# ArielElb/zkSnark-FinalProject

Measured on AMD Instinct MI355X. Metric: groth16_proofs_per_sec, higher is better.
Workload: dtype u32; 1 GPU; matrix-mul 128x128 + Poseidon MatrixCircuit: 10706932 constraints, 8675313 witness vars, domain 2^24; pk/R1CS/assignment resident in HBM; real key (zkg16_setup_resident) with window tables (zkg16_pk_precompute), last timed proof verified (zkg16_verify); parallelism=1 GPU

## Files before the change

__graft_entry__.py:

```python
import os
import subprocess
import sys

ROOT = os.path.dirname(os.path.abspath(__file__))
for p in (ROOT, os.path.join(ROOT, "tests"), os.path.join(ROOT, "tests", "golden"), os.path.join(ROOT, "oracle")):
    if p not in sys.path:
        sys.path.insert(0, p)


def build():
    import importlib.util
    spec = importlib.util.spec_from_file_location("zkg16_build", os.path.join(ROOT, "zksnark-finalproject_amd", "build.py"))
    mod = importlib.util.module_from_spec(spec)
    spec.loader.exec_module(mod)
    mod.build()
    subprocess.check_call(["make", "-C", os.path.join(ROOT, "oracle"), "-s"])
    import prim_cases
    prim_cases.build_shim("host")
    prim_cases.build_shim("device")
    import madd_lazy_cases
    madd_lazy_cases.build_shim("host")
    madd_lazy_cases.build_shim("device")
    import zksnark_finalproject_amd as z
    z.load()
    return None


def smoke():
    import random

    import numpy as np

    import oracle as orc
    import synth
    from helpers import fr_mont, fr_mont_vec
    import pyref as P
    from zksnark_finalproject_amd import Device

    dev = Device(0)
    rng = random.Random(2026)
    nc, ni, nv = 3000, 4, 2500
    A, B, C, z = synth.random_r1cs(rng, nc, ni, nv)
    r1cs = synth.r1cs_arrays(A, B, C, ni)
    pk, _ = synth.make_pk(orc, r1cs, nv, rng, point_gen=dev.fixed_base)
    zm = fr_mont_vec(z)
    r, s = fr_mont(P.rand_fr(rng)), fr_mont(P.rand_fr(rng))
    ph = dev.pk_load(pk, ni)
    proof, inf = dev.prove(ph, r, s, r1cs, zm)
    eproof, einf = orc.prove(pk, r, s, r1cs, zm)
    assert np.array_equal(proof, eproof) and np.array_equal(inf, einf), "HIP proof != oracle proof"
    print("smoke ok: proof bit-identical to the oracle;", dev.last_timings())
    dev.close()
    return None


if __name__ == "__main__":
    build()
    if len(sys.argv) > 1 and sys.argv[1] == "smoke":
        smoke()
```

zksnark-finalproject_amd/build.py:

```python
import os
import subprocess
import sys
from concurrent.futures import ThreadPoolExecutor

HERE = os.path.dirname(os.path.abspath(__file__))
CSRC = os.path.join(HERE, "csrc")
OBJ = os.path.join(HERE, "build")
LIB = os.path.join(HERE, "libzkg16.so")
SOURCES = ["api.hip", "api_keys.hip", "api_prove.hip", "api_stages.hip", "api_group.hip", "api_verify.hip", "api_rerandomize.hip", "api_trapdoor.hip", "ntt.hip", "poly.hip", "msm.hip", "sort.hip", "bucket_sort.hip", "setup.hip", "circuits.hip", "verify.hip", "witness.hip", "matrix_r1cs.hip", "prime_device.hip", "group.hip", "verify_batch.hip"]
HEADERS = ["ff.cuh", "ffu.cuh", "fru.cuh", "ec.cuh", "common.hpp", "api_internal.hpp", "hostff.hpp", "matrix_plan.hpp", "prime_program.hpp", "group.hpp", "verify_batch.hpp", "pairing_dev.cuh", "pairing_each_dev.cuh", "decompress_dev.cuh", "sponge_chain_dev.cuh", "linear_dev.cuh", "linear_elim_dev.cuh", "prime_inputs_dev.cuh", "u64_inputs_dev.cuh", "rerandomize_dev.cuh", "r1cs_check_dev.cuh", "trapdoor_dev.cuh", "pairing_fast.inc", "poseidon_h64.inc", "poseidon_params.inc", "prime_circuit.inc", "final_exp.inc", os.path.join("..", "..", "include", "zkg16.h")]
FLAGS = ["--offload-arch=gfx950", "-O3", "-std=c++17", "-fPIC", "-fvisibility=hidden", "-Wall", "-Wno-unused-function"]


def _stale(target, deps):
    if not os.path.exists(target):
        return True
    t = os.path.getmtime(target)
    return any(os.path.getmtime(d) > t for d in deps)


def build(force=False, verbose=True):
    os.makedirs(OBJ, exist_ok=True)
    hdrs = [os.path.join(CSRC, h) for h in HEADERS] + [os.path.abspath(__file__)]
    jobs = []
    for src in SOURCES:
        s = os.path.join(CSRC, src)
        o = os.path.join(OBJ, src.replace(".hip", ".o"))
        if force or _stale(o, [s] + hdrs):
            jobs.append((s, o))

    def cc(job):
        s, o = job
        cmd = ["hipcc"] + FLAGS + ["-c", s, "-o", o]
        if verbose:
            print(" ".join(cmd), flush=True)
        subprocess.check_call(cmd)

    with ThreadPoolExecutor(max_workers=4) as ex:
        list(ex.map(cc, jobs))
    objs = [os.path.join(OBJ, s.replace(".hip", ".o")) for s in SOURCES]
    if force or jobs or _stale(LIB, objs):
        cmd = ["hipcc", "--offload-arch=gfx950", "-shared", "-fPIC", "-o", LIB] + objs
        if verbose:
            print(" ".join(cmd), flush=True)
        subprocess.check_call(cmd)
    return LIB


if __name__ == "__main__":
    build(force="--force" in sys.argv)
```

zksnark-finalproject_amd/csrc/api.hip:

```cpp
#include "api_internal.hpp"

using namespace zk;

namespace zk {
ScopedKernelTimer::ScopedKernelTimer(zkg16_ctx *c, const char *n, double u, hipStream_t st)
    : ctx(c), name(n), units(u), stream(st ? st : c->stream) {
    if (!ctx->opt.kernel_timing) return;
    if (ctx->opt.kernel_timing_accumulate_only && strncmp(n, "msm_accumulate", 14) != 0) return;
    ZK_HIP(hipEventCreate(&e0));
    ZK_HIP(hipEventCreate(&e1));
    ZK_HIP(hipEventRecord(e0, stream));
}
ScopedKernelTimer::~ScopedKernelTimer() {
    if (!e0) return;
    (void)hipEventRecord(e1, stream);
    ctx->pending_events.push_back(PendingEvent{name, units, e0, e1});
}
void kernel_timer_resolve(zkg16_ctx *ctx) {
    if (ctx->pending_events.empty()) return;
    (void)hipStreamSynchronize(ctx->stream);
    (void)hipStreamSynchronize(ctx->wm_stream);
    for (auto &sl : ctx->slots)
        if (sl.stream) (void)hipStreamSynchronize(sl.stream);
    for (auto &p : ctx->pending_events) {
// ... 278 lines not shown
    if (!ctx) return;
    (void)hipSetDevice(ctx->device);
    for (auto &l : ctx->lanes)
        if (l) {
            {
                std::lock_guard<std::mutex> lk(l->mu);
                teardown(l.get());
            }
            l.reset();
        }
    teardown(ctx);
    ctx->pks.clear();
    ctx->r1cs.clear();
    ctx->wits.clear();
    ctx->prime_dev.reset();
    ctx->ntt_tables.clear();
    delete ctx;
    dev_cache_flush();
}

}
namespace {
int set_option_one(zkg16_ctx *ctx, const char *name, int64_t v) {
    zkg16_ctx::Options &o = ctx->opt;
    const auto is = [name](const char *n) { return !strcmp(name, n); };
    const auto set = [v](int &dst, int64_t lo, int64_t hi, int64_t stored, bool also = true) {
        if (v < lo || v > hi || !also) return (int)ZKG16_ERR_BAD_ARG;
        dst = (int)stored;
        return (int)ZKG16_OK;
    };
    if (is("window_bits")) return set(o.window_bits, 0, 20, v, v != 1);
    if (is("min_seg")) return set(o.min_seg, 0, 4096, v);
    if (is("ntt_mode")) return set(o.ntt_mode, 0, 3, v, v != 2);
    if (is("reduce_mode")) return set(o.reduce_mode, 0, 6, v == 0 ? 3 : v == 4 ? 0 : v);
    if (is("g1_waves")) return set(o.g1_waves, 0, 4, v);
    if (is("fixup_aux")) return set(o.fixup_aux, INT64_MIN, INT64_MAX, v ? 1 : 0);
    if (is("window_bits_h")) return set(o.window_bits_h, 0, 20, v, v != 1);
    if (is("wm_concurrent")) { o.wm_concurrent = (int)v; return ZKG16_OK; }
    if (is("ntt_radix")) return set(o.ntt_radix, 0, 4, v == 0 ? 1 : v);
    if (is("ntt_xcd")) return set(o.ntt_xcd, 0, 2, v == 2 ? 0 : 1);
    if (is("table_stride")) return set(o.table_stride, 0, 2, v);
    if (is("acc_debug")) return set(o.acc_debug, 0, 15, v);
    if (is("sort_mode")) return set(o.sort_mode, 0, 1, v);
    if (is("acc_pipeline")) return set(o.acc_pipeline, 0, 4, v == 4 ? 0 : v);
    if (is("fuse_pointwise")) return set(o.fuse_pointwise, INT64_MIN, INT64_MAX, v ? 1 : 0);
    if (is("wm_transforms")) return set(o.wm_transforms, 0, 7, v == 7 ? 7 : 6, v == 0 || v >= 6);
    if (is("wm_first")) return set(o.wm_first, -1, 2, v);
    if (is("spmv_dict")) return set(o.spmv_dict, 0, 2, v);
    if (is("b_filter")) return set(o.b_filter, 0, 2, v);
    if (is("collect_threads")) return set(o.collect_threads, 0, 2, v == 0 ? -1 : v == 2 ? 0 : 1);
    if (is("fixed_base_bits")) return set(o.fixed_base_bits, 0, 20, v, v == 0 || (v >= 4 && !(v > 14 && (v & 1))));
    if (is("g2_lazy")) return set(o.g2_lazy, 0, 2, v == 2 ? 0 : 1);
    if (is("g1_inline")) return set(o.g1_inline, 0, 2, v == 2 ? 0 : 1);
    if (is("acc_lazy")) return set(o.acc_lazy, 0, 1, v);
    if (is("matrix_parts")) return set(o.matrix_parts, 0, 8, v);
    if (is("matrix_slice_min")) return set(o.matrix_slice_min, 0, 1 << 20, v == 0 ? MATRIX_SLICE_MIN_DEFAULT : v);
    if (is("batch_max")) return set(o.batch_max, 0, 65535, v);
    if (is("matrix_batch_threads")) return set(o.matrix_batch_threads, 0, 16, v);
    if (is("matrix_batch_grid")) return set(o.matrix_batch_grid, 0, 65535, v);
    if (is("linear_solver")) return set(o.linear_solver, 0, 1, v);
    if (is("linear_elim_lds_max")) return set(o.linear_elim_lds_max, 0, 64, v);
    if (is("sponge_chains_min")) {
        if (v < 0) return ZKG16_ERR_BAD_ARG;
        o.sponge_chains_min = v == 0 ? ZKG16_SPONGE_CHAINS_MIN_DEFAULT : v;
        return ZKG16_OK;
    }
    if (is("sponge_chain_segment")) return set(o.sponge_chain_segment, 0, 65535, v);
    if (is("verify_batch_min")) return set(o.verify_batch_min, 0, 1 << 30, v == 0 ? ZKG16_VERIFY_BATCH_MIN_DEFAULT : v);
    if (is("verify_wire_min")) return set(o.verify_wire_min, 0, 1 << 30, v == 0 ? ZKG16_VERIFY_WIRE_MIN_DEFAULT : v);
    if (is("verify_each_after")) {
        const int rc = set(o.verify_each_after, 0, 1 << 30, v == 0 ? ZKG16_VERIFY_EACH_AFTER_DEFAULT : v);
        if (rc == ZKG16_OK) o.verify_each_after_set = v != 0;
        return rc;
    }
    if (is("rerandomize_min")) return set(o.rerandomize_min, 0, 1 << 30, v == 0 ? ZKG16_RERANDOMIZE_MIN_DEFAULT : v);
    if (is("rerandomize_pass")) return set(o.rerandomize_pass, 0, 65536, v);
    if (is("check_satisfied")) return set(o.check_satisfied, 0, 1, v);
    if (is("trapdoor_pass")) return set(o.trapdoor_pass, 0, 65535, v);
    if (is("reduce_chunk")) return set(o.reduce_chunk, 0, 64, v, (v & (v - 1)) == 0);
    return ZKG16_ERR_UNSUPPORTED;
}
}
extern "C" {

int zkg16_set_option(zkg16_ctx *ctx, const char *name, int64_t value) {
    if (!ctx || !name) return ZKG16_ERR_BAD_ARG;
    if (!strcmp(name, "lanes")) {
        if (value < 1 || value > 8) return ZKG16_ERR_BAD_ARG;
        std::lock_guard<std::mutex> lk(ctx->lane_mu);
        ctx->opt_lanes = (int)value;
        return ZKG16_OK;
    }
    int rc;
    {
        std::lock_guard<std::mutex> lk(ctx->mu);
        rc = set_option_one(ctx, name, value);
    }
    if (rc != ZKG16_OK) return rc;
    std::vector<zkg16_ctx *> ls;
    {
        std::lock_guard<std::mutex> lk(ctx->lane_mu);
        for (auto &l : ctx->lanes)
            if (l) ls.push_back(l.get());
    }
    for (zkg16_ctx *l : ls) {
        std::lock_guard<std::mutex> lk(l->mu);
// ... 174 lines not shown
```

zksnark-finalproject_amd/csrc/common.hpp:

```cpp
#pragma once
#include <hip/hip_runtime.h>
#include <stdint.h>
#include <stdio.h>
#include <string.h>

#include <algorithm>
#include <array>
#include <atomic>
#include <condition_variable>
#include <functional>
#include <map>
#include <memory>
#include <mutex>
#include <shared_mutex>
#include <string>
#include <system_error>
#include <thread>
#include <vector>

#include "../../include/zkg16.h"
#include "ec.cuh"
#include "ff.cuh"

namespace zk {
// ... 218 lines not shown
    zkg16_ctx *root = nullptr;
    std::unique_ptr<zkg16_ctx> lanes[7];
    std::mutex lane_mu;
    std::condition_variable lane_cv;
    bool lane_busy[8] = {false, false, false, false, false, false, false, false};
    int opt_lanes = 2;
    int last_lane = 0;
    std::shared_mutex key_rw;
    struct LaneLogEntry { int lane; double t0_ms, t1_ms; };
    std::vector<LaneLogEntry> lane_log;
    zk::MsmWorkspace ws_z, ws_h, ws_zb;
    hipStream_t wm_stream = nullptr;
    zk::MsmSlot slots[5];
    int last_msm_group = 0;
    void *extra_host = nullptr;
    void *stage_host[2] = {nullptr, nullptr};
    hipEvent_t stage_done[2] = {nullptr, nullptr};
    zk::DevBuf poly[4];
    void *batch_host = nullptr;
    size_t batch_host_bytes = 0;
    bool batch_terms_set = false;
    uint64_t batch_terms[3] = {0, 0, 0};
    void *mbatch_host = nullptr;
    size_t mbatch_host_bytes = 0;
    zk::DevBuf mbatch_dev;
    zk::DevBuf check_dev;
    std::vector<uint64_t> check_n_bad, check_first_bad;
    float timings[zk::PROOF_TIMING_SLOTS] = {0};
    struct Options {
        bool kernel_timing = false;
        bool kernel_timing_accumulate_only = false;
        int window_bits = 0;
        int min_seg = 0;
        int ntt_mode = 1;
        int reduce_mode = 3;
        int b_filter = 0;
        int spmv_dict = 0;
        int wm_first = -1;
        int g1_waves = 0;
        int fixup_aux = 0;
        int window_bits_h = 0;
        int reduce_chunk = 0;
        int wm_concurrent = -1;
        int ntt_radix = 1;
        int ntt_xcd = 1;
        int table_stride = 0;
        int acc_debug = 0;
        int sort_mode = 0;
        int acc_pipeline = 0;
        int collect_threads = -1;
        int fixed_base_bits = 0;
        int g2_lazy = 1;
        int acc_lazy = 1;
        int g1_inline = 1;
        int matrix_parts = 0;
        int matrix_slice_min = MATRIX_SLICE_MIN_DEFAULT;
        int fuse_pointwise = 1;
        int wm_transforms = 6;
        int batch_max = 0;
        int matrix_batch_threads = 0;
        int matrix_batch_grid = 0;
        int linear_solver = 0;
        int linear_elim_lds_max = 0;
        int64_t sponge_chains_min = ZKG16_SPONGE_CHAINS_MIN_DEFAULT;
        int sponge_chain_segment = 0;
        int verify_batch_min = ZKG16_VERIFY_BATCH_MIN_DEFAULT;
        int verify_wire_min = ZKG16_VERIFY_WIRE_MIN_DEFAULT;
        int check_satisfied = 0;
        int verify_each_after = ZKG16_VERIFY_EACH_AFTER_DEFAULT;
        int rerandomize_min = ZKG16_RERANDOMIZE_MIN_DEFAULT;
        int rerandomize_pass = 0;
        int trapdoor_pass = 0;
        int verify_each_after_set = 0;
    } opt;
    std::map<std::string, zk::KernelStat> kstats;
    std::vector<zk::PendingEvent> pending_events;
    void *circuit_stage = nullptr;
    size_t circuit_stage_bytes = 0;
    float vb_timings[zk::VERIFY_TIMING_SLOTS] = {0};
    float rr_timings[zk::RERANDOMIZE_TIMING_SLOTS] = {0};
    int num_cus = 256;
    bool lds_attr_fixup[2] = {false, false}, lds_attr_ntt = false, lds_attr_linear_elim = false;
    zk::FixedBaseCache fb_g1, fb_g2;
    zk::DevBuf poseidon_dev;
    std::shared_ptr<zk::PrimeDev> prime_dev;
};

namespace zk {

struct PendingEvent { std::string name; double units; hipEvent_t e0, e1; };

struct ScopedKernelTimer {
    zkg16_ctx *ctx;
    const char *name;
    double units;
    hipEvent_t e0 = nullptr, e1 = nullptr;
    hipStream_t stream;
    ScopedKernelTimer(zkg16_ctx *c, const char *n, double u, hipStream_t st = nullptr);
    ~ScopedKernelTimer();
};
void kernel_timer_resolve(zkg16_ctx *ctx);

struct NttPointwise { const Fr *b, *c; Fr zinv; };
struct NttLast { const Fr *scale; bool pw_operand, sub; };
Fr *ntt_run(zkg16_ctx *ctx, Fr *src, Fr *dst, int log_n, bool inverse, bool coset, const NttPointwise *pw = nullptr,
            const NttLast *last = nullptr);
// ... 151 lines not shown
```

zksnark-finalproject_amd/csrc/msm.hip:

```cpp
#include <chrono>

#include "common.hpp"

namespace zk {

template <class F> struct FieldTraits;
template <> struct FieldTraits<FqU> { using Sat = Fq; static constexpr bool g2 = false; };
template <> struct FieldTraits<Fq2U> { using Sat = Fq2; static constexpr bool g2 = true; };
template <> struct FieldTraits<Fq> { using Sat = Fq; static constexpr bool g2 = false; };
template <> struct FieldTraits<Fq2> { using Sat = Fq2; static constexpr bool g2 = true; };

template <class T>
__device__ __forceinline__ T ldv(const T *p) {
    static_assert(sizeof(T) % 16 == 0, "16-byte multiple");
    T v;
    const uint4 *q = reinterpret_cast<const uint4 *>(p);
    uint4 *d = reinterpret_cast<uint4 *>(&v);
#pragma unroll
    for (unsigned i = 0; i < sizeof(T) / 16; i++) d[i] = q[i];
    return v;
}
template <class T>
__device__ __forceinline__ void stv(T *p, const T &v) {
    uint4 *q = reinterpret_cast<uint4 *>(p);
    const uint4 *s = reinterpret_cast<const uint4 *>(&v);
#pragma unroll
    for (unsigned i = 0; i < sizeof(T) / 16; i++) q[i] = s[i];
}

struct DigitSrc {
    const uint32_t *scalars, *extra;
    size_t n_main, n;
    const uint8_t *mask;
    int mont;
    const uint8_t *part;
    int want;
    const uint32_t *const *vecs;
    size_t vec_stride;
};
__global__ void __launch_bounds__(256) msm_digits_kernel(DigitSrc src, int c, int nwin, size_t nb, uint64_t *keys, uint32_t *codes, uint32_t invalid_bucket) {
    const size_t i = (size_t)blockIdx.x * blockDim.x + threadIdx.x;
    const size_t n = src.n;
    if (i >= n) return;
    const unsigned v = blockIdx.y;
    const uint32_t *mainv = src.vecs ? src.vecs[v] : src.scalars + (size_t)v * src.vec_stride * 8;
    const uint32_t *extrav = src.extra + (size_t)v * (n - src.n_main) * 8;
    const size_t w0 = (size_t)v * nwin;
    uint32_t s[9];
    {
        const uint4 *q = reinterpret_cast<const uint4 *>(i < src.n_main ? mainv + 8 * i : extrav + 8 * (i - src.n_main));
        uint4 lo = q[0], hi = q[1];
        if (src.mask && src.mask[i]) lo = hi = make_uint4(0, 0, 0, 0);
        if (src.part && (int)src.part[i] != src.want) lo = hi = make_uint4(0, 0, 0, 0);
        Fr v;
        v.l[0] = lo.x; v.l[1] = lo.y; v.l[2] = lo.z; v.l[3] = lo.w; v.l[4] = hi.x; v.l[5] = hi.y; v.l[6] = hi.z; v.l[7] = hi.w;
// ... 189 lines not shown
                    head_b = (int32_t)cur;
                    dst = a.seg_head + t;
                } else if (!acc.is_inf()) {
                    dst = a.buckets + cur;
                }
                if (dst != nullptr && !(a.debug & 1u)) stv(dst, acc);
                acc = XYZZ<F>::inf();
                cur = gb;
            }
            const Affine<F> b = bq;
            en = en1;
            en1 = a.entries[p + 2 < end ? p + 2 : end - 1];
            bq = ld_base<F>(bases, (a.debug & 2u) ? 0u : (a.debug & 4u) ? ((en.x >> 1) & 0xffffu) : (en.x >> 1));
            __builtin_amdgcn_sched_barrier(0);
            if constexpr (LC) xyzz_madd_inline_lc(acc, b, (e & 1u) != 0);
            else xyzz_madd_inline(acc, b, (e & 1u) != 0);
        }
    } else {
        uint32_t e = en.x, gb = en.y;
        for (uint32_t p = start; p < end; p++) {
            if (p + 1 < end) en = a.entries[p + 1];
            const uint32_t e_n = en.x, g_n = en.y;
            if (gb != cur) {
                if (cur == g_first && head_open) {
                    head_b = (int32_t)cur;
                    stv(a.seg_head + t, acc);
                } else if (!acc.is_inf()) {
                    stv(a.buckets + cur, acc);
                }
                acc = XYZZ<F>::inf();
                cur = gb;
            }
            const Affine<F> b = ld_base<F>(bases, e >> 1);
            if constexpr (LAZY && LC && FieldTraits<F>::g2) xyzz_madd_lazy_lc(acc, b, (e & 1u) != 0);
            else if constexpr (LAZY && FieldTraits<F>::g2) xyzz_madd_lazy(acc, b, (e & 1u) != 0);
            else xyzz_madd(acc, b, (e & 1u) != 0);
            e = e_n;
            gb = g_n;
        }
    }
    if (cur == g_first && head_open) {
        head_b = (int32_t)cur;
        stv(a.seg_head + t, acc);
    } else if (cur == g_after) {
        tail_b = (int32_t)cur;
        stv(a.seg_tail + t, acc);
    } else if (!acc.is_inf()) {
        stv(a.buckets + cur, acc);
    }
    a.seg_meta[2 * t] = head_b;
    a.seg_meta[2 * t + 1] = tail_b;
}

static constexpr int FIXUP_SHORT = 4;
static constexpr uint32_t FIXUP_ITEM = 1024;
struct FixQueue {
    uint32_t *counts;
    uint2 *items;
    uint4 *chains;
};

template <class F>
__global__ void __launch_bounds__(64) msm_fixup_kernel(AccArgs<F> a, FixQueue q) {
    const size_t t = (size_t)blockIdx.x * blockDim.x + threadIdx.x;
    const size_t seg_len = *a.seg_len_ptr;
    if (t * seg_len >= (size_t)*a.total_ptr) return;
    const int32_t g = a.seg_meta[2 * t + 1];
    if (g < 0) return;
    const size_t last_seg = ((size_t)a.offsets[g + 1] - 1) / seg_len;
    if (last_seg - t > FIXUP_SHORT) {
        const uint32_t n_items = (uint32_t)((last_seg - t + FIXUP_ITEM - 1) / FIXUP_ITEM);
        const uint32_t base = atomicAdd(q.counts, n_items);
        for (uint32_t j = 0; j < n_items; j++) q.items[base + j] = make_uint2((uint32_t)t, j);
        if (n_items > 1) q.chains[atomicAdd(q.counts + 1, 1u)] = make_uint4((uint32_t)t, base, n_items, 0u);
        return;
    }
    XYZZ<F> sum = ldv(a.seg_tail + t);
    for (size_t u = t + 1; u <= last_seg; u++) {
        const XYZZ<F> h = ldv(a.seg_head + u);
        xyzz_add(sum, h);
    }
    stv(a.buckets + g, sum);
}

template <class F>
__device__ __forceinline__ void block_fold(XYZZ<F> *sh, const XYZZ<F> &mine) {
    sh[threadIdx.x] = mine;
    __syncthreads();
    for (int d = 128; d >= 1; d >>= 1) {
        if ((int)threadIdx.x < d) {
            XYZZ<F> x = sh[threadIdx.x];
            const XYZZ<F> y = sh[threadIdx.x + d];
            xyzz_add(x, y);
            sh[threadIdx.x] = x;
        }
        __syncthreads();
    }
}

template <class F>
__global__ void __launch_bounds__(256) msm_fixup_long_kernel(AccArgs<F> a, FixQueue q, XYZZ<F> *item_sums) {
    extern __shared__ __attribute__((aligned(16))) unsigned char fix_smem[];
    XYZZ<F> *sh = reinterpret_cast<XYZZ<F> *>(fix_smem);
    const uint32_t n_items = q.counts[0];
    for (uint32_t item = blockIdx.x; item < n_items; item += gridDim.x) {
        const size_t t = q.items[item].x, j = q.items[item].y;
// ... 486 lines not shown
__global__ void __launch_bounds__(256) zero_fill_kernel(uint4 *p, size_t n16, uint32_t *also) {
    const size_t i = (size_t)blockIdx.x * blockDim.x + threadIdx.x;
    if (i < n16) p[i] = make_uint4(0, 0, 0, 0);
    if (i == 0 && also) also[0] = also[1] = 0;
}
static void zero_fill(hipStream_t st, void *p, size_t bytes, uint32_t *also) {
    const size_t n16 = bytes / 16;
    hipLaunchKernelGGL(zero_fill_kernel, dim3((unsigned)((n16 + 255) / 256)), dim3(256), 0, st, reinterpret_cast<uint4 *>(p), n16, also);
}

template <class F>
static FixQueue fix_queue(MsmSlot &slot, size_t nseg) {
    const size_t cap_items = nseg + 16, cap_chains = nseg / FIXUP_ITEM + 16;
    slot.long_list.ensure(16 + cap_items * sizeof(uint2) + cap_chains * sizeof(uint4));
    slot.long_sums.ensure(cap_items * sizeof(XYZZ<F>));
    unsigned char *p = slot.long_list.as<unsigned char>();
    return FixQueue{reinterpret_cast<uint32_t *>(p), reinterpret_cast<uint2 *>(p + 16), reinterpret_cast<uint4 *>(p + 16 + cap_items * sizeof(uint2))};
}
template <class F>
static void msm_launch_fixups(zkg16_ctx *ctx, MsmSlot &slot, hipStream_t fs) {
    AccArgs<F> a;
    memcpy(&a, slot.acc_args, sizeof a);
    const size_t psz = sizeof(XYZZ<F>);
    const FixQueue q = fix_queue<F>(slot, (size_t)slot.acc_grid * 64);
    XYZZ<F> *sums = slot.long_sums.as<XYZZ<F>>();
    {
        ScopedKernelTimer kt(ctx, FieldTraits<F>::g2 ? "msm_fixup_g2" : "msm_fixup_g1", (double)slot.acc_grid * 64, fs);
        hipLaunchKernelGGL(msm_fixup_kernel<F>, dim3(slot.acc_grid), dim3(64), 0, fs, a, q);
    }
    bool &lds_attr_set = ctx->lds_attr_fixup[FieldTraits<F>::g2 ? 1 : 0];
    if (!lds_attr_set) {
        ZK_HIP(hipFuncSetAttribute(reinterpret_cast<const void *>(msm_fixup_long_kernel<F>), hipFuncAttributeMaxDynamicSharedMemorySize, 160 * 1024));
        ZK_HIP(hipFuncSetAttribute(reinterpret_cast<const void *>(msm_fixup_fold_kernel<F>), hipFuncAttributeMaxDynamicSharedMemorySize, 160 * 1024));
        lds_attr_set = true;
    }
    {
        ScopedKernelTimer kt(ctx, FieldTraits<F>::g2 ? "msm_fixup_long_g2" : "msm_fixup_long_g1", 0.0, fs);
        hipLaunchKernelGGL(msm_fixup_long_kernel<F>, dim3(512), dim3(256), 256 * psz, fs, a, q, sums);
        hipLaunchKernelGGL(msm_fixup_fold_kernel<F>, dim3(64), dim3(256), 256 * psz, fs, a, q, sums);
    }
}

template <class F>
__global__ void __launch_bounds__(64, FieldTraits<F>::g2 ? 1 : 2) msm_bucket_merge_kernel(XYZZ<F> *sum, const XYZZ<F> *add, size_t n) {
    const size_t i = (size_t)blockIdx.x * blockDim.x + threadIdx.x;
    if (i >= n) return;
    const XYZZ<F> b = ldv(add + i);
    if (b.is_inf()) return;
    XYZZ<F> a = ldv(sum + i);
    xyzz_add(a, b);
    stv(sum + i, a);
}

template <class F, class BASE>
static void msm_launch_accumulate(zkg16_ctx *ctx, unsigned grid, const AccArgs<F> &a) {
    const bool pipe = (ctx->opt.acc_pipeline >> (FieldTraits<F>::g2 ? 1 : 0)) & 1;
    const bool lc = ctx->opt.acc_lazy != 0;
    if (pipe) {
        hipLaunchKernelGGL((msm_accumulate_kernel<F, BASE, true>), dim3(grid), dim3(64), 0, ctx->stream, a);
    } else if constexpr (FieldTraits<F>::g2) {
        if (ctx->opt.g2_lazy && lc) hipLaunchKernelGGL((msm_accumulate_kernel<F, BASE, false, true, false, true>), dim3(grid), dim3(64), 0, ctx->stream, a);
        else if (ctx->opt.g2_lazy) hipLaunchKernelGGL((msm_accumulate_kernel<F, BASE, false, true>), dim3(grid), dim3(64), 0, ctx->stream, a);
        else hipLaunchKernelGGL((msm_accumulate_kernel<F, BASE, false>), dim3(grid), dim3(64), 0, ctx->stream, a);
    } else {
        if (!ctx->opt.g1_inline) hipLaunchKernelGGL((msm_accumulate_kernel<F, BASE, false, false, true>), dim3(grid), dim3(64), 0, ctx->stream, a);
        else if (lc) hipLaunchKernelGGL((msm_accumulate_kernel<F, BASE, false, false, false, true>), dim3(grid), dim3(64), 0, ctx->stream, a);
        else hipLaunchKernelGGL((msm_accumulate_kernel<F, BASE, false>), dim3(grid), dim3(64), 0, ctx->stream, a);
    }
}

template <class F>
static void msm_enqueue_acc(zkg16_ctx *ctx, MsmWorkspace &ws, const MsmPlan &plan, const Affine<F> *bases, MsmSlot &slot, int round = -1, bool padded = false) {
    if (round <= 0) {
        slot.active = false;
        slot.pending_reduce = false;
    }
    slot.nwin = plan.nwin;
    slot.c = plan.c;
    slot.batch = plan.batch;
    if (plan.n == 0) return;
    const size_t tb = plan.nb * plan.nwin;
    const size_t psz = sizeof(XYZZ<F>);
    if (!slot.acc_done) {
        ZK_HIP(hipEventCreate(&slot.acc_done));
        ZK_HIP(hipEventCreate(&slot.red_done));
        ZK_HIP(hipEventCreate(&slot.acc_start));
        ZK_HIP(hipEventCreate(&slot.red_start));
        if (!slot.stream) ZK_HIP(hipStreamCreateWithFlags(&slot.stream, hipStreamNonBlocking));
    }
    if (round <= 0) ZK_HIP(hipEventRecord(slot.acc_start, ctx->stream));
    XYZZ<F> *target;
    if (round == 0) {
        slot.bucket_sum.ensure(tb * psz);
        target = slot.bucket_sum.as<XYZZ<F>>();
    } else {
        slot.buckets.ensure(tb * psz);
        target = slot.buckets.as<XYZZ<F>>();
    }
    const size_t nseg = FieldTraits<F>::g2 ? plan.lanes_g2 : plan.lanes_g1;
    slot.seg_head.ensure(nseg * psz);
    slot.seg_tail.ensure(nseg * psz);
    slot.seg_meta.ensure(nseg * 2 * sizeof(int32_t));
    const FixQueue fq = fix_queue<F>(slot, (nseg + 63) / 64 * 64);
    zero_fill(ctx->stream, target, tb * psz, fq.counts);
    AccArgs<F> a;
    a.bases = bases;
    a.entries = ws.entries.as<uint2>();
    a.offsets = ws.offsets.as<uint32_t>();
    a.buckets = target;
    a.seg_head = slot.seg_head.as<XYZZ<F>>();
// ... 150 lines not shown
template <class FS>
static XYZZ<FS> msm_combine(const MsmSlot &slot, int w0, int nw) {
    const XYZZ<FS> *wsum = reinterpret_cast<const XYZZ<FS> *>(slot.wsums_host);
    auto window = [&](int w) {
        if (slot.bit_sliced) {
            const int bits = slot.bit_sliced;
            XYZZ<FS> v = wsum[(bits + 1) * slot.nwin + w];
            for (int t = bits - 1; t >= 0; t--) {
                v = xyzz_dbl(v);
                xyzz_add(v, wsum[t * slot.nwin + w]);
            }
            for (int k = slot.two_level_k; k > 1; k >>= 1) v = xyzz_dbl(v);
            xyzz_add(v, xyzz_neg(wsum[bits * slot.nwin + w]));
            return v;
        }
        if (!slot.two_level_k) return wsum[w];
        XYZZ<FS> v = wsum[w];
        for (int k = slot.two_level_k; k > 1; k >>= 1) v = xyzz_dbl(v);
        xyzz_add(v, xyzz_neg(wsum[slot.nwin + w]));
        return v;
    };
    XYZZ<FS> total = window(w0 + nw - 1);
    for (int w = w0 + nw - 2; w >= w0; w--) {
        for (int q = 0; q < slot.c; q++) total = xyzz_dbl(total);
        xyzz_add(total, window(w));
    }
    return total;
}
template <class FS>
static XYZZ<FS> msm_collect(zkg16_ctx *ctx, MsmSlot &slot) {
    (void)ctx;
    if (!slot.active) return XYZZ<FS>::inf();
    ZK_HIP(hipEventSynchronize(slot.red_done));
    const auto host_t0 = std::chrono::steady_clock::now();
    struct Lap { const std::chrono::steady_clock::time_point t0; MsmSlot &s; ~Lap() { s.collect_host_ms = std::chrono::duration<float, std::milli>(std::chrono::steady_clock::now() - t0).count(); } } lap{host_t0, slot};
    const XYZZ<FS> total = msm_combine<FS>(slot, 0, slot.nwin);
    slot.active = false;
    return total;
}
template <class FS>
static XYZZ<FS> msm_collect_part(const MsmSlot &slot, int v) {
    if (!slot.active) return XYZZ<FS>::inf();
    const int nw = slot.nwin / (slot.batch > 1 ? slot.batch : 1);
    return msm_combine<FS>(slot, v * nw, nw);
}
void msm_slot_wait(MsmSlot &slot) {
    if (slot.active) ZK_HIP(hipEventSynchronize(slot.red_done));
}

int msm_acc_resident_waves(zkg16_ctx *ctx, bool g2) {
    int blocks = 0;
    const bool pipe = (ctx->opt.acc_pipeline >> (g2 ? 1 : 0)) & 1;
    hipError_t e;
    if (g2) {
        if (pipe) e = hipOccupancyMaxActiveBlocksPerMultiprocessor(&blocks, msm_accumulate_kernel<Fq2U, Affine<Fq2U>, true>, 64, 0);
        else if (ctx->opt.g2_lazy && ctx->opt.acc_lazy) e = hipOccupancyMaxActiveBlocksPerMultiprocessor(&blocks, msm_accumulate_kernel<Fq2U, Affine<Fq2U>, false, true, false, true>, 64, 0);
        else if (ctx->opt.g2_lazy) e = hipOccupancyMaxActiveBlocksPerMultiprocessor(&blocks, msm_accumulate_kernel<Fq2U, Affine<Fq2U>, false, true>, 64, 0);
        else e = hipOccupancyMaxActiveBlocksPerMultiprocessor(&blocks, msm_accumulate_kernel<Fq2U, Affine<Fq2U>, false>, 64, 0);
    } else {
        if (pipe) e = hipOccupancyMaxActiveBlocksPerMultiprocessor(&blocks, msm_accumulate_kernel<FqU, Affine<FqU>, true>, 64, 0);
        else if (!ctx->opt.g1_inline) e = hipOccupancyMaxActiveBlocksPerMultiprocessor(&blocks, msm_accumulate_kernel<FqU, Affine<FqU>, false, false, true>, 64, 0);
        else if (ctx->opt.acc_lazy) e = hipOccupancyMaxActiveBlocksPerMultiprocessor(&blocks, msm_accumulate_kernel<FqU, Affine<FqU>, false, false, false, true>, 64, 0);
        else e = hipOccupancyMaxActiveBlocksPerMultiprocessor(&blocks, msm_accumulate_kernel<FqU, Affine<FqU>, false>, 64, 0);
    }
    ZK_HIP(e);
    return blocks / 4;
}

void msm_g1_enqueue_acc(zkg16_ctx *ctx, MsmWorkspace &ws, const MsmPlan &plan, const G1AffineU *bases, MsmSlot &slot, int round, bool padded) { msm_enqueue_acc<FqU>(ctx, ws, plan, bases, slot, round, padded); }
void msm_g2_enqueue_acc(zkg16_ctx *ctx, MsmWorkspace &ws, const MsmPlan &plan, const G2AffineU *bases, MsmSlot &slot, int round, bool padded) { msm_enqueue_acc<Fq2U>(ctx, ws, plan, bases, slot, round, padded); }
void msm_g1_enqueue_reduce(zkg16_ctx *ctx, MsmSlot &slot) { msm_enqueue_reduce<FqU>(ctx, slot); }
void msm_g2_enqueue_reduce(zkg16_ctx *ctx, MsmSlot &slot) { msm_enqueue_reduce<Fq2U>(ctx, slot); }
void msm_g1_enqueue(zkg16_ctx *ctx, MsmWorkspace &ws, const MsmPlan &plan, const G1AffineU *bases, MsmSlot &slot, bool padded) { msm_enqueue<FqU>(ctx, ws, plan, bases, slot, padded); }
void msm_g2_enqueue(zkg16_ctx *ctx, MsmWorkspace &ws, const MsmPlan &plan, const G2AffineU *bases, MsmSlot &slot, bool padded) { msm_enqueue<Fq2U>(ctx, ws, plan, bases, slot, padded); }
G1XYZZ msm_g1_collect(zkg16_ctx *ctx, MsmSlot &slot) { return msm_collect<Fq>(ctx, slot); }
G2XYZZ msm_g2_collect(zkg16_ctx *ctx, MsmSlot &slot) { return msm_collect<Fq2>(ctx, slot); }
G1XYZZ msm_g1_collect_part(const MsmSlot &slot, int v) { return msm_collect_part<Fq>(slot, v); }
G2XYZZ msm_g2_collect_part(const MsmSlot &slot, int v) { return msm_collect_part<Fq2>(slot, v); }

G1XYZZ msm_g1_exec(zkg16_ctx *ctx, MsmWorkspace &ws, const MsmPlan &plan, const G1AffineU *bases, const char *tag) {
    (void)tag;
    msm_enqueue<FqU>(ctx, ws, plan, bases, ctx->slots[0]);
    return msm_collect<Fq>(ctx, ctx->slots[0]);
}
G2XYZZ msm_g2_exec(zkg16_ctx *ctx, MsmWorkspace &ws, const MsmPlan &plan, const G2AffineU *bases, const char *tag) {
    (void)tag;
    msm_enqueue<Fq2U>(ctx, ws, plan, bases, ctx->slots[0]);
    return msm_collect<Fq2>(ctx, ctx->slots[0]);
}
void convert_g1_bases(zkg16_ctx *ctx, const G1Affine *in, G1AffineU *out, size_t n) {
    if (!n) return;
    hipLaunchKernelGGL(convert_bases_kernel<FqU>, dim3((unsigned)((n + 255) / 256)), dim3(256), 0, ctx->stream, in, out, n);
    ZK_HIP(hipGetLastError());
}
void convert_g2_bases(zkg16_ctx *ctx, const G2Affine *in, G2AffineU *out, size_t n) {
    if (!n) return;
    hipLaunchKernelGGL(convert_bases_kernel<Fq2U>, dim3((unsigned)((n + 255) / 256)), dim3(256), 0, ctx->stream, in, out, n);
    ZK_HIP(hipGetLastError());
}

template <class FU>
static void batch_affine_run(zkg16_ctx *ctx, const XYZZ<FU> *pts, size_t n, DevBuf &pref, const AffineSegs<FU> &segs) {
    size_t threads = (size_t)ctx->num_cus * 4 * 64;
    if (threads * 4 > n) threads = (n + 3) / 4;
    const unsigned blocks = (unsigned)((threads + 63) / 64);
    pref.ensure(n * sizeof(FU));
    hipLaunchKernelGGL(batch_affine_kernel<FU>, dim3(blocks), dim3(64), 0, ctx->stream, pts, n, pref.as<FU>(), segs);
// ... 164 lines not shown
```

Baseline: 7.246 proofs/s.

## Split G2 bucket accumulation across lane pairs, one Fq component per lane

Adds a G2 MSM accumulate kernel in which each Fq2 point is handled by two adjacent lanes, each holding one Fq component. Fq2 multiplies are built from lane-partner exchanges via DPP swaps. It launches twice the grid, is on by default, and defaults to the lazy/inline form. The aim is to cut per-thread register pressure and raise occupancy and parallelism for the G2 bucket accumulation, at the cost of cross-lane shuffles and some duplicated control flow.

```diff
diff --git a/__graft_entry__.py b/__graft_entry__.py
--- a/__graft_entry__.py
+++ b/__graft_entry__.py
@@ -21,6 +21,8 @@
     import madd_lazy_cases
     madd_lazy_cases.build_shim("host")
     madd_lazy_cases.build_shim("device")
+    import g2_split_cases
+    g2_split_cases.build_shim()
     import zksnark_finalproject_amd as z
     z.load()
     return None
diff --git a/zksnark-finalproject_amd/build.py b/zksnark-finalproject_amd/build.py
--- a/zksnark-finalproject_amd/build.py
+++ b/zksnark-finalproject_amd/build.py
@@ -8,7 +8,7 @@
 OBJ = os.path.join(HERE, "build")
 LIB = os.path.join(HERE, "libzkg16.so")
 SOURCES = ["api.hip", "api_keys.hip", "api_prove.hip", "api_stages.hip", "api_group.hip", "api_verify.hip", "api_rerandomize.hip", "api_trapdoor.hip", "ntt.hip", "poly.hip", "msm.hip", "sort.hip", "bucket_sort.hip", "setup.hip", "circuits.hip", "verify.hip", "witness.hip", "matrix_r1cs.hip", "prime_device.hip", "group.hip", "verify_batch.hip"]
-HEADERS = ["ff.cuh", "ffu.cuh", "fru.cuh", "ec.cuh", "common.hpp", "api_internal.hpp", "hostff.hpp", "matrix_plan.hpp", "prime_program.hpp", "group.hpp", "verify_batch.hpp", "pairing_dev.cuh", "pairing_each_dev.cuh", "decompress_dev.cuh", "sponge_chain_dev.cuh", "linear_dev.cuh", "linear_elim_dev.cuh", "prime_inputs_dev.cuh", "u64_inputs_dev.cuh", "rerandomize_dev.cuh", "r1cs_check_dev.cuh", "trapdoor_dev.cuh", "pairing_fast.inc", "poseidon_h64.inc", "poseidon_params.inc", "prime_circuit.inc", "final_exp.inc", os.path.join("..", "..", "include", "zkg16.h")]
+HEADERS = ["ff.cuh", "ffu.cuh", "fru.cuh", "ec.cuh", "g2split.cuh", "common.hpp", "api_internal.hpp", "hostff.hpp", "matrix_plan.hpp", "prime_program.hpp", "group.hpp", "verify_batch.hpp", "pairing_dev.cuh", "pairing_each_dev.cuh", "decompress_dev.cuh", "sponge_chain_dev.cuh", "linear_dev.cuh", "linear_elim_dev.cuh", "prime_inputs_dev.cuh", "u64_inputs_dev.cuh", "rerandomize_dev.cuh", "r1cs_check_dev.cuh", "trapdoor_dev.cuh", "pairing_fast.inc", "poseidon_h64.inc", "poseidon_params.inc", "prime_circuit.inc", "final_exp.inc", os.path.join("..", "..", "include", "zkg16.h")]
 FLAGS = ["--offload-arch=gfx950", "-O3", "-std=c++17", "-fPIC", "-fvisibility=hidden", "-Wall", "-Wno-unused-function"]
 
 
diff --git a/zksnark-finalproject_amd/csrc/api.hip b/zksnark-finalproject_amd/csrc/api.hip
--- a/zksnark-finalproject_amd/csrc/api.hip
+++ b/zksnark-finalproject_amd/csrc/api.hip
@@ -354,6 +354,8 @@
     if (is("fixed_base_bits")) return set(o.fixed_base_bits, 0, 20, v, v == 0 || (v >= 4 && !(v > 14 && (v & 1))));
     if (is("g2_lazy")) return set(o.g2_lazy, 0, 2, v == 2 ? 0 : 1);
     if (is("g1_inline")) return set(o.g1_inline, 0, 2, v == 2 ? 0 : 1);
+    if (is("g2_split")) return set(o.g2_split, 0, 1, v);
+    if (is("g2_split_form")) return set(o.g2_split_form, 0, 2, v == 2 ? 0 : v);
     if (is("acc_lazy")) return set(o.acc_lazy, 0, 1, v);
     if (is("matrix_parts")) return set(o.matrix_parts, 0, 8, v);
     if (is("matrix_slice_min")) return set(o.matrix_slice_min, 0, 1 << 20, v == 0 ? MATRIX_SLICE_MIN_DEFAULT : v);
diff --git a/zksnark-finalproject_amd/csrc/common.hpp b/zksnark-finalproject_amd/csrc/common.hpp
--- a/zksnark-finalproject_amd/csrc/common.hpp
+++ b/zksnark-finalproject_amd/csrc/common.hpp
@@ -294,6 +294,8 @@
         int fixed_base_bits = 0;
         int g2_lazy = 1;
         int acc_lazy = 1;
+        int g2_split = 1;
+        int g2_split_form = 0;
         int g1_inline = 1;
         int matrix_parts = 0;
         int matrix_slice_min = MATRIX_SLICE_MIN_DEFAULT;
diff --git a/zksnark-finalproject_amd/csrc/g2split.cuh b/zksnark-finalproject_amd/csrc/g2split.cuh
--- /dev/null
+++ b/zksnark-finalproject_amd/csrc/g2split.cuh
@@ -0,0 +1,238 @@
+#pragma once
+#include "ec.cuh"
+
+namespace zk {
+
+template <bool INL>
+struct H2Lane {
+    using V = FqU;
+    using B = bool;
+    static constexpr bool INLINE = INL;
+    int h;
+    ZK_HD static uint32_t swap_u32(uint32_t v) {
+#if defined(__HIP_DEVICE_COMPILE__)
+        return (uint32_t)__builtin_amdgcn_update_dpp(0, (int)v, 0xB1, 0xF, 0xF, false);
+#else
+        return v;
+#endif
+    }
+    ZK_HD V partner(const V &a) const {
+        V r;
+#pragma unroll
+        for (int i = 0; i < 14; i++) r.l[i] = swap_u32(a.l[i]);
+        return r;
+    }
+    ZK_HD V by_parity(const V &odd, const V &even) const {
+        V r;
+#pragma unroll
+        for (int i = 0; i < 14; i++) r.l[i] = h ? odd.l[i] : even.l[i];
+        return r;
+    }
+    ZK_HD bool both(bool mine) const { return mine && swap_u32(mine ? 1u : 0u) != 0u; }
+    template <class Fn, class... A> ZK_HD V each(Fn f, const A &...a) const { return f(a...); }
+    template <class Fn, class... A> ZK_HD B test(Fn f, const A &...a) const { return f(a...); }
+    ZK_HD V one() const {
+        V r;
+#pragma unroll
+        for (int i = 0; i < 14; i++) r.l[i] = h ? 0u : FqUP::one(i);
+        return r;
+    }
+};
+
+#if !defined(__HIP_DEVICE_COMPILE__)
+struct H2PairV { FqU c[2]; };
+struct H2PairB { bool c[2]; };
+struct H2Pair {
+    using V = H2PairV;
+    using B = H2PairB;
+    static constexpr bool INLINE = true;
+    V partner(const V &a) const { return V{{a.c[1], a.c[0]}}; }
+    V by_parity(const V &odd, const V &even) const { return V{{even.c[0], odd.c[1]}}; }
+    bool both(const B &p) const { return p.c[0] && p.c[1]; }
+    template <class Fn, class... A> V each(Fn f, const A &...a) const { return V{{f(a.c[0]...), f(a.c[1]...)}}; }
+    template <class Fn, class... A> B test(Fn f, const A &...a) const { return B{{f(a.c[0]...), f(a.c[1]...)}}; }
+    V one() const { return V{{FqU::one(), FqU::zero()}}; }
+};
+#endif
+
+template <class M> ZK_HD typename M::V h2_zero(const M &m) { return m.each([]() { return FqU::zero(); }); }
+template <class M> ZK_HD typename M::V h2_add(const M &m, const typename M::V &a, const typename M::V &b) {
+    return m.each([](const FqU &x, const FqU &y) { return fqu_add(x, y); }, a, b);
+}
+template <class M> ZK_HD typename M::V h2_dbl(const M &m, const typename M::V &a) { return h2_add(m, a, a); }
+template <int L, class M> ZK_HD typename M::V h2_sub(const M &m, const typename M::V &a, const typename M::V &b) {
+    return m.each([](const FqU &x, const FqU &y) { return fqu_sub<L>(x, y); }, a, b);
+}
+template <class M> ZK_HD typename M::V h2_neg(const M &m, const typename M::V &a) {
+    return m.each([](const FqU &x) { return fqu_neg(x); }, a);
+}
+template <class M> ZK_HD bool h2_is_zero(const M &m, const typename M::V &a) {
+    return m.both(m.test([](const FqU &x) { return x.is_zero(); }, a));
+}
+template <class M> ZK_HD bool h2_is_zero_mod(const M &m, const typename M::V &a) {
+    return m.both(m.test([](const FqU &x) { return fqu_is_zero_mod(x); }, a));
+}
+
+template <bool LC, class M> ZK_HD typename M::V h2_mul_body(const M &m, const typename M::V &a, const typename M::V &b) {
+    using V = typename M::V;
+    const V nb = m.each([](const FqU &x) { return LC ? fqu_rsub_raw<128>(x) : fqu_sub<128>(FqU::zero(), x); }, b);
+    const V pb = m.partner(m.by_parity(nb, b)), pa = m.partner(a);
+    const V mine = m.by_parity(pa, a), theirs = m.by_parity(a, pa);
+    return m.each([](const FqU &x, const FqU &y, const FqU &z, const FqU &w) { return fqu_mul2_lc<LC ? 30 : 29>(x, y, z, w); }, mine, b, pb, theirs);
+}
+template <bool LC, class M> ZK_HD typename M::V h2_sqr_operand_x(const M &m, const typename M::V &a, const typename M::V &pa) {
+    return m.by_parity(pa, m.each([](const FqU &x, const FqU &y) { return LC ? fqu_add_raw(x, y) : fqu_add(x, y); }, a, pa));
+}
+template <class M> ZK_HD typename M::V h2_sqr_operand_y(const M &m, const typename M::V &a, const typename M::V &pa) {
+    return m.by_parity(a, h2_sub<128>(m, a, pa));
+}
+template <class M> ZK_HD typename M::V h2_sqr_finish(const M &m, const typename M::V &r) {
+    return h2_add(m, r, m.by_parity(r, h2_zero(m)));
+}
+
+#if defined(__HIP_DEVICE_COMPILE__)
+template <bool LC>
+__device__ __noinline__ FqURet h2_mul_call(zk_v4u a0, zk_v4u a1, zk_v4u a2, zk_v2u a3, zk_v4u b0, zk_v4u b1, zk_v4u b2, zk_v2u b3, int h) {
+    FqU a, b;
+    a.l[0] = a0.x; a.l[1] = a0.y; a.l[2] = a0.z; a.l[3] = a0.w; a.l[4] = a1.x; a.l[5] = a1.y; a.l[6] = a1.z; a.l[7] = a1.w;
+    a.l[8] = a2.x; a.l[9] = a2.y; a.l[10] = a2.z; a.l[11] = a2.w; a.l[12] = a3.x; a.l[13] = a3.y;
+    b.l[0] = b0.x; b.l[1] = b0.y; b.l[2] = b0.z; b.l[3] = b0.w; b.l[4] = b1.x; b.l[5] = b1.y; b.l[6] = b1.z; b.l[7] = b1.w;
+    b.l[8] = b2.x; b.l[9] = b2.y; b.l[10] = b2.z; b.l[11] = b2.w; b.l[12] = b3.x; b.l[13] = b3.y;
+    const FqU r = h2_mul_body<LC>(H2Lane<false>{h}, a, b);
+    FqURet o;
+#pragma unroll
+    for (int i = 0; i < 14; i++) o.l[i] = r.l[i];
+    return o;
+}
+#endif
+
+template <bool LC, class M> ZK_HD typename M::V h2_mul(const M &m, const typename M::V &a, const typename M::V &b) {
+#if defined(__HIP_DEVICE_COMPILE__)
+    if constexpr (!M::INLINE) {
+        zk_v4u a0 = {a.l[0], a.l[1], a.l[2], a.l[3]}, a1 = {a.l[4], a.l[5], a.l[6], a.l[7]}, a2 = {a.l[8], a.l[9], a.l[10], a.l[11]};
+        zk_v2u a3 = {a.l[12], a.l[13]};
+        zk_v4u b0 = {b.l[0], b.l[1], b.l[2], b.l[3]}, b1 = {b.l[4], b.l[5], b.l[6], b.l[7]}, b2 = {b.l[8], b.l[9], b.l[10], b.l[11]};
+        zk_v2u b3 = {b.l[12], b.l[13]};
+        const FqURet r = h2_mul_call<LC>(a0, a1, a2, a3, b0, b1, b2, b3, m.h);
+        FqU o;
+#pragma unroll
+        for (int i = 0; i < 14; i++) o.l[i] = r.l[i];
+        return o;
+    } else {
+        __builtin_amdgcn_sched_barrier(0);
+        const typename M::V r = h2_mul_body<LC>(m, a, b);
+        __builtin_amdgcn_sched_barrier(0);
+        return r;
+    }
+#else
+    return h2_mul_body<LC>(m, a, b);
+#endif
+}
+template <bool LC, class M> ZK_HD typename M::V h2_sqr(const M &m, const typename M::V &a) {
+    using V = typename M::V;
+    const V pa = m.partner(a);
+    const V x = h2_sqr_operand_x<LC>(m, a, pa), y = h2_sqr_operand_y(m, a, pa);
+    V r;
+#if defined(__HIP_DEVICE_COMPILE__)
+    if constexpr (!M::INLINE) r = fqu_mul(x, y);
+    else r = fqu_mul_il(x, y);
+#else
+    r = m.each([](const FqU &s, const FqU &t) { return fqu_mul_impl<false, LC ? 30 : 29, 29>(s, t); }, x, y);
+#endif
+    return h2_sqr_finish(m, r);
+}
+
+template <class M> struct H2Affine { typename M::V x, y; };
+template <class M> struct H2XYZZ { typename M::V x, y, zz, zzz; };
+
+template <class M> ZK_HD H2XYZZ<M> h2_inf(const M &m) { return H2XYZZ<M>{h2_zero(m), h2_zero(m), h2_zero(m), h2_zero(m)}; }
+template <class M> ZK_HD bool h2_is_inf(const M &m, const H2XYZZ<M> &p) { return h2_is_zero(m, p.zz); }
+template <class M> ZK_HD bool h2_is_inf(const M &m, const H2Affine<M> &p) {
+    return m.both(m.test([](const FqU &x, const FqU &y) { return x.is_zero() && y.is_zero(); }, p.x, p.y));
+}
+
+template <class M> ZK_HD H2XYZZ<M> h2_dbl_affine(const M &m, const H2Affine<M> &q) {
+    using V = typename M::V;
+    const V U = h2_dbl(m, q.y);
+    const V Vv = h2_sqr<false>(m, U);
+    const V W = h2_mul<false>(m, U, Vv);
+    const V S = h2_mul<false>(m, q.x, Vv);
+    const V X2 = h2_sqr<false>(m, q.x);
+    const V Mm = h2_add(m, h2_dbl(m, X2), X2);
+    H2XYZZ<M> r;
+    r.x = h2_sub<32>(m, h2_sqr<false>(m, Mm), h2_dbl(m, S));
+    r.y = h2_sub<32>(m, h2_mul<false>(m, Mm, h2_sub<64>(m, S, r.x)), h2_mul<false>(m, W, q.y));
+    r.zz = Vv;
+    r.zzz = W;
+    return r;
+}
+
+template <bool LC, class M> ZK_HD bool h2_madd_nd(const M &m, H2XYZZ<M> &acc, const H2Affine<M> &q, bool neg) {
+    using V = typename M::V;
+    if (h2_is_inf(m, q)) return true;
+    if (h2_is_inf(m, acc)) {
+        acc = H2XYZZ<M>{q.x, neg ? h2_neg(m, q.y) : q.y, m.one(), m.one()};
+        return true;
+    }
+    const V U2 = h2_mul<LC>(m, q.x, acc.zz);
+    V R;
+    if constexpr (LC) {
+        const V S2 = h2_mul<LC>(m, q.y, acc.zzz);
+        R = m.each([neg](const FqU &s, const FqU &y) { return fqu_addsub_sel(s, fqu_rsub_raw<64>(y), neg); }, S2, acc.y);
+    } else {
+        const V S2 = h2_mul<LC>(m, neg ? h2_neg(m, q.y) : q.y, acc.zzz);
+        R = h2_sub<64>(m, S2, acc.y);
+    }
+    const V Pp = h2_sub<64>(m, U2, acc.x);
+    if (h2_is_zero_mod(m, Pp)) {
+        if (h2_is_zero_mod(m, R)) return false;
+        acc = h2_inf(m);
+        return true;
+    }
+    const V PP = h2_sqr<LC>(m, Pp);
+    const V PPP = h2_mul<LC>(m, Pp, PP);
+    acc.zz = h2_mul<LC>(m, acc.zz, PP);
+    acc.zzz = h2_mul<LC>(m, acc.zzz, PPP);
+    const V Q = h2_mul<LC>(m, acc.x, PP);
+    const V RR = h2_sqr<LC>(m, R);
+    V X3;
+    if constexpr (LC) X3 = m.each([](const FqU &rr, const FqU &b, const FqU &c) { return fqu_sub_b_2c(rr, b, c); }, RR, PPP, Q);
+    else X3 = h2_sub<32>(m, RR, h2_add(m, PPP, h2_dbl(m, Q)));
+    const V T = h2_mul<LC>(m, R, h2_sub<64>(m, Q, X3));
+    acc.y = h2_sub<32>(m, T, h2_mul<LC>(m, acc.y, PPP));
+    acc.x = X3;
+    return true;
+}
+template <class M> ZK_HD H2XYZZ<M> h2_dbl_term(const M &m, const H2Affine<M> &q, bool neg) {
+    return h2_dbl_affine(m, H2Affine<M>{q.x, neg ? h2_neg(m, q.y) : q.y});
+}
+template <bool LC, class M> ZK_HD void h2_madd(const M &m, H2XYZZ<M> &acc, const H2Affine<M> &q, bool neg) {
+    if (!h2_madd_nd<LC>(m, acc, q, neg)) acc = h2_dbl_term(m, q, neg);
+}
+
+__device__ __forceinline__ FqU h2_ld(const FqU *p) {
+    const uint2 *q = reinterpret_cast<const uint2 *>(p);
+    FqU v;
+#pragma unroll
+    for (int i = 0; i < 7; i++) { const uint2 w = q[i]; v.l[2 * i] = w.x; v.l[2 * i + 1] = w.y; }
+    return v;
+}
+__device__ __forceinline__ void h2_st(FqU *p, const FqU &v) {
+    uint2 *q = reinterpret_cast<uint2 *>(p);
+#pragma unroll
+    for (int i = 0; i < 7; i++) q[i] = make_uint2(v.l[2 * i], v.l[2 * i + 1]);
+}
+template <class M> __device__ __forceinline__ H2Affine<M> h2_ld_affine(const M &m, const Affine<Fq2U> *p) {
+    const FqU *f = reinterpret_cast<const FqU *>(p);
+    return H2Affine<M>{h2_ld(f + m.h), h2_ld(f + 2 + m.h)};
+}
+template <class M> __device__ __forceinline__ H2XYZZ<M> h2_ld_xyzz(const M &m, const XYZZ<Fq2U> *p) {
+    const FqU *f = reinterpret_cast<const FqU *>(p);
+    return H2XYZZ<M>{h2_ld(f + m.h), h2_ld(f + 2 + m.h), h2_ld(f + 4 + m.h), h2_ld(f + 6 + m.h)};
+}
+template <class M> __device__ __forceinline__ void h2_st_xyzz(const M &m, XYZZ<Fq2U> *p, const H2XYZZ<M> &v) {
+    FqU *f = reinterpret_cast<FqU *>(p);
+    h2_st(f + m.h, v.x); h2_st(f + 2 + m.h, v.y); h2_st(f + 4 + m.h, v.zz); h2_st(f + 6 + m.h, v.zzz);
+}
+
+}
diff --git a/zksnark-finalproject_amd/csrc/msm.hip b/zksnark-finalproject_amd/csrc/msm.hip
--- a/zksnark-finalproject_amd/csrc/msm.hip
+++ b/zksnark-finalproject_amd/csrc/msm.hip
@@ -1,6 +1,7 @@
 #include <chrono>
 
 #include "common.hpp"
+#include "g2split.cuh"
 
 namespace zk {
 
@@ -296,6 +297,61 @@
     a.seg_meta[2 * t + 1] = tail_b;
 }
 
+template <class F> __device__ __forceinline__ const Affine<F> *base_ptr(const Affine<F> *b, uint32_t i) { return b + i; }
+template <class F> __device__ __forceinline__ const Affine<F> *base_ptr(const PadAffine<F> *b, uint32_t i) { return &b[i].p; }
+
+template <class BASE, bool LC, bool INL>
+__global__ void __launch_bounds__(64, 2) msm_accumulate_split_kernel(AccArgs<Fq2U> a) {
+    using M = H2Lane<INL>;
+    const BASE *const bases = static_cast<const BASE *>(a.bases);
+    const uint32_t t = (blockIdx.x * 64u + threadIdx.x) >> 1;
+    const M m{(int)(threadIdx.x & 1u)};
+    const uint32_t total = *a.total_ptr;
+    const uint32_t seg_len = *a.seg_len_ptr;
+    const uint32_t start = t * seg_len;
+    if (start >= total) return;
+    const uint32_t end = start + seg_len < total ? start + seg_len : total;
+    uint2 en = a.entries[start];
+    const uint32_t g_first = en.y;
+    const bool head_open = start > 0 && a.entries[start - 1].y == g_first;
+    const uint32_t g_after = end < total ? a.entries[end].y : 0xffffffffu;
+    int32_t head_b = -1, tail_b = -1;
+    H2XYZZ<M> acc = h2_inf(m);
+    uint32_t cur = g_first;
+    uint32_t e = en.x, gb = en.y;
+    for (uint32_t p = start; p < end; p++) {
+        if (p + 1 < end) en = a.entries[p + 1];
+        const uint32_t e_n = en.x, g_n = en.y;
+        if (gb != cur) {
+            if (cur == g_first && head_open) {
+                head_b = (int32_t)cur;
+                h2_st_xyzz(m, a.seg_head + t, acc);
+            } else if (!h2_is_inf(m, acc)) {
+                h2_st_xyzz(m, a.buckets + cur, acc);
+            }
+            acc = h2_inf(m);
+            cur = gb;
+        }
+        const H2Affine<M> b = h2_ld_affine(m, base_ptr(bases, e >> 1));
+        if (!h2_madd_nd<LC>(m, acc, b, (e & 1u) != 0)) acc = h2_dbl_term(m, h2_ld_affine(m, base_ptr(bases, e >> 1)), (e & 1u) != 0);
+        e = e_n;
+        gb = g_n;
+    }
+    if (cur == g_first && head_open) {
+        head_b = (int32_t)cur;
+        h2_st_xyzz(m, a.seg_head + t, acc);
+    } else if (cur == g_after) {
+        tail_b = (int32_t)cur;
+        h2_st_xyzz(m, a.seg_tail + t, acc);
+    } else if (!h2_is_inf(m, acc)) {
+        h2_st_xyzz(m, a.buckets + cur, acc);
+    }
+    if (m.h == 0) {
+        a.seg_meta[2 * t] = head_b;
+        a.seg_meta[2 * t + 1] = tail_b;
+    }
+}
+
 static constexpr int FIXUP_SHORT = 4;
 static constexpr uint32_t FIXUP_ITEM = 1024;
 struct FixQueue {
@@ -888,10 +944,26 @@
     stv(sum + i, a);
 }
 
+static bool g2_split_on(const zkg16_ctx *ctx) { return ctx->opt.g2_split && ctx->opt.g2_lazy && !(ctx->opt.acc_pipeline & 2) && !ctx->opt.acc_debug; }
+static int g2_split_form(const zkg16_ctx *ctx) {
+    if (!ctx->opt.acc_lazy) return 0;
+    return ctx->opt.g2_split_form == 1 ? 1 : 2;
+}
+
 template <class F, class BASE>
 static void msm_launch_accumulate(zkg16_ctx *ctx, unsigned grid, const AccArgs<F> &a) {
     const bool pipe = (ctx->opt.acc_pipeline >> (FieldTraits<F>::g2 ? 1 : 0)) & 1;
     const bool lc = ctx->opt.acc_lazy != 0;
+    if constexpr (FieldTraits<F>::g2) {
+        if (g2_split_on(ctx)) {
+            switch (g2_split_form(ctx)) {
+                case 0: hipLaunchKernelGGL((msm_accumulate_split_kernel<BASE, false, false>), dim3(2 * grid), dim3(64), 0, ctx->stream, a); break;
+                case 1: hipLaunchKernelGGL((msm_accumulate_split_kernel<BASE, true, false>), dim3(2 * grid), dim3(64), 0, ctx->stream, a); break;
+                default: hipLaunchKernelGGL((msm_accumulate_split_kernel<BASE, true, true>), dim3(2 * grid), dim3(64), 0, ctx->stream, a); break;
+            }
+            return;
+        }
+    }
     if (pipe) {
         hipLaunchKernelGGL((msm_accumulate_kernel<F, BASE, true>), dim3(grid), dim3(64), 0, ctx->stream, a);
     } else if constexpr (FieldTraits<F>::g2) {
@@ -1148,7 +1220,13 @@
     int blocks = 0;
     const bool pipe = (ctx->opt.acc_pipeline >> (g2 ? 1 : 0)) & 1;
     hipError_t e;
-    if (g2) {
+    if (g2 && g2_split_on(ctx)) {
+        switch (g2_split_form(ctx)) {
+            case 0: e = hipOccupancyMaxActiveBlocksPerMultiprocessor(&blocks, msm_accumulate_split_kernel<Affine<Fq2U>, false, false>, 64, 0); break;
+            case 1: e = hipOccupancyMaxActiveBlocksPerMultiprocessor(&blocks, msm_accumulate_split_kernel<Affine<Fq2U>, true, false>, 64, 0); break;
+            default: e = hipOccupancyMaxActiveBlocksPerMultiprocessor(&blocks, msm_accumulate_split_kernel<Affine<Fq2U>, true, true>, 64, 0); break;
+        }
+    } else if (g2) {
         if (pipe) e = hipOccupancyMaxActiveBlocksPerMultiprocessor(&blocks, msm_accumulate_kernel<Fq2U, Affine<Fq2U>, true>, 64, 0);
         else if (ctx->opt.g2_lazy && ctx->opt.acc_lazy) e = hipOccupancyMaxActiveBlocksPerMultiprocessor(&blocks, msm_accumulate_kernel<Fq2U, Affine<Fq2U>, false, true, false, true>, 64, 0);
         else if (ctx->opt.g2_lazy) e = hipOccupancyMaxActiveBlocksPerMultiprocessor(&blocks, msm_accumulate_kernel<Fq2U, Affine<Fq2U>, false, true>, 64, 0);
```

New measurement: 7.595 proofs/s, median of 6. 4.8% higher.
